# uzh-rpg/rpg_ramnet

Measured on AMD Instinct MI355X. Metric: depth samples/sec (346x260 cropped to 256x344, 5-bin grids, K=5 grids + 1 frame per sample; training step), higher is better.
Workload: dtype f32; 1 GPU; EventScape-shaped 346x260 -> 256x344 crop, 5 event bins, K=5, batch 8/GPU, seq-len 8, 1xMI355X-per-rank train, state=convgru, SI loss on [image,events4], Adam, backward-weights co-scheduled on a side stream, decoders on a second stream; global_batch=8, seq_len=8, parallelism=dp1

## Files before the change

rpg_ramnet_amd/csrc/conv_wgrad_wino24.hip:

```cpp
#include <stdlib.h>
#include "common.hpp"

namespace ramnet {

constexpr int G24_T = 8;

struct Wgrad24Params {
    const float *x, *g, *gm;
    float *dw, *dbias;
    int ldx, ldg, ldgm, Hp, Wp, H2, W2, Hc, Wc, Cin, Cout, tiles_x, tiles_y, ntiles, nbatch, ncob;
    size_t xbytes, gbytes, gmbytes;
};

template <bool GM, bool WCI>
__global__ void __launch_bounds__(512, 1) conv_wgrad_wino24_kernel(const Wgrad24Params p) {
    constexpr int G24_CI = WCI ? 64 : 32, G24_CO = WCI ? 32 : 64;
    constexpr int G24_V = 25 * G24_T * G24_CI, G24_Z = 25 * G24_T * G24_CO;
    extern __shared__ __attribute__((aligned(16))) float smem[];
    float *V = smem;
    float *Z = smem + 2 * G24_V;
    const int tid = threadIdx.x, lane = tid & 63;
    const int wave = __builtin_amdgcn_readfirstlane(tid >> 6);
    const int l31 = lane & 31, kk = lane >> 5;
    const int pg = wave >> 1, ch = wave & 1;
    const int p0 = pg == 0 ? 0 : 1 + 6 * pg;
    const int cls = blockIdx.z / p.ncob, cob = blockIdx.z % p.ncob;
    const int py = cls >> 1, px = cls & 1;
    const int c0 = blockIdx.y * G24_CI, n0 = cob * G24_CO;
    const bool vrole = WCI || wave < 4, zrole = !WCI || wave < 4;
    const int vt = (tid / G24_CI) & 7, vc = tid % G24_CI;
    const int zt = (tid / G24_CO) & 7, zc = tid % G24_CO;

    f32x16 acc[7];
#pragma unroll
    for (int i = 0; i < 7; ++i)
#pragma unroll
        for (int r = 0; r < 16; ++r) acc[i][r] = 0.f;

    float vraw[25], zraw[4];
    float bsum = 0.f;
    struct Walk { int tx, ty, b, T; };
    const int dT = G24_T * (int)gridDim.x;
    const int d_tx = dT % p.tiles_x, d_ty = (dT / p.tiles_x) % p.tiles_y, d_b = (dT / p.tiles_x) / p.tiles_y;
    auto walk_init = [&](Walk &w, int batch, int tile) {
        w.T = batch * G24_T + tile;
        int t = w.T;
        w.tx = t % p.tiles_x;
        t /= p.tiles_x;
        w.ty = t % p.tiles_y, w.b = t / p.tiles_y;
    };
    auto walk_step = [&](Walk &w, int adv) {
        w.T += adv * dT;
        w.tx += adv * d_tx;
        const int cx = w.tx >= p.tiles_x ? 1 : 0;
        w.tx -= cx * p.tiles_x;
        w.ty += adv * d_ty + cx;
        const int cy = w.ty >= p.tiles_y ? 1 : 0;
        w.ty -= cy * p.tiles_y;
        w.b += adv * d_b + cy;
    };
    Walk wv, wz;
    int lbv = 0, lbz = 0;
    const auto rx = wino_rsrc(p.x, (unsigned)min((size_t)p.xbytes, (size_t)WOOB));
    const auto rg = wino_rsrc(p.g, (unsigned)min((size_t)p.gbytes, (size_t)WOOB));
    const auto rgm = GM ? wino_rsrc(p.gm, (unsigned)min((size_t)p.gmbytes, (size_t)WOOB)) : rg;
    const bool vch_ok = c0 + vc < p.Cin, zch_ok = n0 + zc < p.Cout;
    const unsigned zch = (unsigned)(n0 + zc);
    const int rowB = p.Wp * p.ldx * 4, colB = p.ldx * 4;
    auto load_v = [&](int batch) {
        walk_step(wv, batch != lbv ? 1 : 0);
        lbv = batch;
        const unsigned base = (unsigned)(((wv.b * p.Hp + 2 * wv.ty + py) * p.Wp + 2 * wv.tx + px) * p.ldx + c0 + vc) * 4u;
        const unsigned lane_off = ((wv.T < p.ntiles) & vch_ok) ? base : WOOB;
#pragma unroll
        for (int r = 0; r < 5; ++r)
#pragma unroll
            for (int c = 0; c < 5; ++c)
                vraw[r * 5 + c] = __builtin_bit_cast(float, __builtin_amdgcn_raw_buffer_load_b32(rx, (int)(lane_off + (unsigned)(r * rowB)), c * colB, 0));
    };
    auto load_z = [&](int batch, bool count) {
        walk_step(wz, batch != lbz ? 1 : 0);
        lbz = batch;
        const bool tok = (wz.T < p.ntiles) & zch_ok;
#pragma unroll
        for (int a = 0; a < 2; ++a)
#pragma unroll
            for (int c = 0; c < 2; ++c) {
                const int oy = 2 * wz.ty + a, ox = 2 * wz.tx + c;
                const bool ok = tok & (oy < p.Hc) & (ox < p.Wc);
                const unsigned pix = (unsigned)((wz.b * p.H2 + 2 * oy + py) * p.W2 + 2 * ox + px);
                float v = __builtin_bit_cast(float, __builtin_amdgcn_raw_buffer_load_b32(rg, (int)(ok ? (pix * p.ldg + zch) * 4u : WOOB), 0, 0));
                if (GM) {
                    const float m = __builtin_bit_cast(float, __builtin_amdgcn_raw_buffer_load_b32(rgm, (int)(ok ? (pix * p.ldgm + zch) * 4u : WOOB), 0, 0));
                    v = m > 0.f ? v : 0.f;
                }
                zraw[a * 2 + c] = v;
                if (count) bsum += v;
            }
    };
    auto v_cols = [&]() {
#pragma unroll
        for (int c = 0; c < 5; ++c) {
            const float d0 = vraw[c], d1 = vraw[5 + c], d2 = vraw[10 + c], d3 = vraw[15 + c], d4 = vraw[20 + c];
            vraw[c] = 2.f * (d0 - d2) - d1 + d3;
            vraw[5 + c] = d3 - d2 - 2.f * d1;
            vraw[10 + c] = 2.f * d1 - 3.f * d2 + d3;
            vraw[15 + c] = d3 - d1;
            vraw[20 + c] = 2.f * (d1 - d3) - d2 + d4;
        }
    };
    auto v_row = [&](float *vbuf, int i) {
        const float d0 = vraw[i * 5], d1 = vraw[i * 5 + 1], d2 = vraw[i * 5 + 2], d3 = vraw[i * 5 + 3], d4 = vraw[i * 5 + 4];
        float *dst = vbuf + ((i * 5) * G24_T + vt) * G24_CI + vc;
        dst[0 * G24_T * G24_CI] = 2.f * (d0 - d2) - d1 + d3;
        dst[1 * G24_T * G24_CI] = d3 - d2 - 2.f * d1;
        dst[2 * G24_T * G24_CI] = 2.f * d1 - 3.f * d2 + d3;
        dst[3 * G24_T * G24_CI] = d3 - d1;
        dst[4 * G24_T * G24_CI] = 2.f * (d1 - d3) - d2 + d4;
    };
    auto z_row = [&](float *zbuf, int i) {
        float w0, w1;
        if (i == 0) w0 = zraw[0], w1 = zraw[1];
        if (i == 1) w0 = zraw[0] + zraw[2], w1 = zraw[1] + zraw[3];
        if (i == 2) w0 = zraw[0] - zraw[2], w1 = zraw[1] - zraw[3];
        if (i == 3) w0 = zraw[0] + 2.f * zraw[2], w1 = zraw[1] + 2.f * zraw[3];
        if (i == 4) w0 = zraw[2], w1 = zraw[3];
        float *dst = zbuf + ((i * 5) * G24_T + zt) * G24_CO + zc;
        dst[0 * G24_T * G24_CO] = w0;
        dst[1 * G24_T * G24_CO] = w0 + w1;
        dst[2 * G24_T * G24_CO] = w0 - w1;
        dst[3 * G24_T * G24_CO] = w0 + 2.f * w1;
        dst[4 * G24_T * G24_CO] = w1;
    };

    const int step = gridDim.x;
    int batch = blockIdx.x;
    if (batch < p.nbatch) {
        const int last = batch + ((p.nbatch - 1 - batch) / step) * step;
        walk_init(wv, batch, vt), walk_init(wz, batch, zt);
        lbv = lbz = batch;
        if (zrole) load_z(batch, true);
        if (vrole) load_v(batch);
        if (zrole) {
#pragma unroll
            for (int i = 0; i < 5; ++i) z_row(Z, i);
        }
        if (vrole) {
            v_cols();
#pragma unroll
            for (int i = 0; i < 5; ++i) v_row(V, i);
        }
        {
            const bool more = batch + step <= last;
            if (zrole) load_z(min(batch + step, last), more);
            if (vrole) load_v(min(batch + step, last));
        }
        __syncthreads();
        const int aoff = (kk * 4) * G24_CI + (WCI ? ch * 32 : 0) + l31, boff = (kk * 4) * G24_CO + (WCI ? 0 : ch * 32) + l31;
        int buf = 0;
        for (; batch <= last; batch += step, buf ^= 1) {
            const float *vb = V + buf * G24_V, *zb = Z + buf * G24_Z;
            float *vn = V + (buf ^ 1) * G24_V, *zn = Z + (buf ^ 1) * G24_Z;
            const int b2 = min(batch + 2 * step, last);
            const bool more2 = batch + 2 * step <= last;
#pragma unroll
            for (int q = 0; q < 7; ++q) {
                if (q < 6 || pg == 0) {
                    const int pos = p0 + q;
                    const float *ap = vb + pos * (G24_T * G24_CI) + aoff, *bp = zb + pos * (G24_T * G24_CO) + boff;
                    const float a0 = ap[0], a1 = ap[G24_CI], a2 = ap[2 * G24_CI], a3 = ap[3 * G24_CI];
                    const float b0 = bp[0], b1 = bp[G24_CO], b2v = bp[2 * G24_CO], b3 = bp[3 * G24_CO];
                    __builtin_amdgcn_sched_barrier(0);
                    acc[q] = __builtin_amdgcn_mfma_f32_32x32x2f32(a0, b0, acc[q], 0, 0, 0);
                    acc[q] = __builtin_amdgcn_mfma_f32_32x32x2f32(a1, b1, acc[q], 0, 0, 0);
                    __builtin_amdgcn_sched_barrier(0);
                    if (q == 0 && zrole) z_row(zn, 0), z_row(zn, 1), z_row(zn, 2);
                    if (q == 1 && zrole) z_row(zn, 3), z_row(zn, 4);
                    if (q == 2 && vrole) v_cols();
                    if (q == 3 && vrole) v_row(vn, 0), v_row(vn, 1), v_row(vn, 2);
                    if (q == 4 && vrole) v_row(vn, 3), v_row(vn, 4);
                    if (q == 4) {
                        if (zrole) load_z(b2, more2);
                        if (vrole) load_v(b2);
                    }
                    __builtin_amdgcn_sched_barrier(0);
                    acc[q] = __builtin_amdgcn_mfma_f32_32x32x2f32(a2, b2v, acc[q], 0, 0, 0);
                    acc[q] = __builtin_amdgcn_mfma_f32_32x32x2f32(a3, b3, acc[q], 0, 0, 0);
                    __builtin_amdgcn_sched_barrier(0);
                }
            }
            __syncthreads();
        }
    }

    const int n = n0 + (WCI ? 0 : ch * 32) + l31;
#pragma unroll
    for (int q = 0; q < 7; ++q) {
        if (q < 6 || pg == 0) {
#pragma unroll
            for (int r = 0; r < 16; ++r) {
                const int c = c0 + (WCI ? ch * 32 : 0) + (r & 3) + 8 * (r >> 2) + 4 * kk;
                if (c < p.Cin && n < p.Cout) atomicAdd(p.dw + (((size_t)cls * 25 + p0 + q) * p.Cin + c) * p.Cout + n, acc[q][r]);
            }
        }
    }
    if (p.dbias != nullptr && blockIdx.y == 0) {
        __syncthreads();
        float *red = smem;
        if (zrole) red[zt * G24_CO + zc] = bsum;
        __syncthreads();
        if (tid < G24_CO) {
            float t = 0.f;
            for (int g = 0; g < 8; ++g) t += red[g * G24_CO + tid];
            if (n0 + tid < p.Cout) atomicAdd(p.dbias + n0 + tid, t);
        }
    }
}

int launch_wgrad_wino24(const ramnet_wgrad_desc &d, hipStream_t st) {
    const bool wci = d.Cout % 64 != 0;
    const int G24_CI = wci ? 64 : 32, G24_CO = wci ? 32 : 64;
    RAMNET_CHECK_ARG(d.in_mode == RAMNET_IN_PLAIN && d.stride == 1 && d.C0 % G24_CI == 0 && d.Cout % 32 == 0);
    RAMNET_CHECK_ARG(d.Hin == d.Ho + 4 && d.Win == d.Wo + 4 && d.HoG == 2 * d.Ho && d.WoG == 2 * d.Wo && d.Ho >= 2 && d.Wo >= 2);
    Wgrad24Params q;
    q.x = d.x0, q.g = d.dout, q.gm = d.gmask, q.dw = d.dw, q.dbias = d.dbias;
    q.ldx = d.ld0, q.ldg = d.ldg, q.ldgm = d.ldgm, q.Hp = d.Hin, q.Wp = d.Win, q.H2 = d.HoG, q.W2 = d.WoG, q.Hc = d.Ho, q.Wc = d.Wo;
    q.Cin = d.C0, q.Cout = d.Cout;
    q.xbytes = (size_t)d.B * d.Hin * d.Win * d.ld0 * 4, q.gbytes = (size_t)d.B * d.HoG * d.WoG * d.ldg * 4;
    q.gmbytes = d.gmask ? (size_t)d.B * d.HoG * d.WoG * d.ldgm * 4 : 0;
    RAMNET_CHECK_ARG(2 * q.xbytes < WOOB && 2 * q.gbytes < WOOB && 2 * q.gmbytes < WOOB);
    q.tiles_x = cdiv(d.Wo, 2), q.tiles_y = cdiv(d.Ho, 2), q.ntiles = q.tiles_x * q.tiles_y * d.B, q.nbatch = cdiv(q.ntiles, G24_T);
    q.ncob = cdiv(d.Cout, G24_CO);
    const int gy = d.C0 / G24_CI, gz = q.ncob * 4;
    int splits = 256 / (gy * gz);
    if (splits > q.nbatch) splits = q.nbatch;
    if (splits < 1) splits = 1;
    const size_t lds = (size_t)2 * 25 * G24_T * (32 + 64) * sizeof(float);
    const dim3 grid(splits, gy, gz);
    auto go = [&](auto kern) -> int {
        RAMNET_FULL_LDS((kern));
        note_kernel("conv_wgrad_wino24_kernel<%d,%d>", d.gmask ? 1 : 0, (int)wci);
        hipLaunchKernelGGL(kern, grid, dim3(512), lds, st, q);
        return 0;
    };
    const int rc = wci ? (d.gmask ? go(conv_wgrad_wino24_kernel<true, true>) : go(conv_wgrad_wino24_kernel<false, true>))
                       : (d.gmask ? go(conv_wgrad_wino24_kernel<true, false>) : go(conv_wgrad_wino24_kernel<false, false>));
    if (rc) return rc;
    RAMNET_LAUNCH_CHECK();
    return 0;
}

}
```

Measured before the change: 247.5 samples/s.

## Software-pipeline LDS operand prefetch and spread transform stages across MFMA slots

Restructures the Winograd F(2,3) weight-gradient main loop so the LDS operands for the next group of MFMAs are fetched into registers ahead of time. The global-load and transform work (z/v loads, column/row transforms, mask application) is split into fine-grained slots interleaved between individual MFMAs instead of coarse chunks. The mid-loop barrier moves so the next buffer's reads overlap the current compute, and LDS base offsets are held as swapped opaque registers. It also adds compile-time ablation macros for profiling. The aim is to hide LDS and global latency behind MFMA issue, at the cost of more register pressure and scheduling complexity.

```diff
diff --git a/rpg_ramnet_amd/csrc/conv_wgrad_wino24.hip b/rpg_ramnet_amd/csrc/conv_wgrad_wino24.hip
--- a/rpg_ramnet_amd/csrc/conv_wgrad_wino24.hip
+++ b/rpg_ramnet_amd/csrc/conv_wgrad_wino24.hip
@@ -1,5 +1,21 @@
 #include <stdlib.h>
+#include <type_traits>
 #include "common.hpp"
+
+#ifndef RAMNET_ABL24
+#define RAMNET_ABL24 0
+#endif
+#define ABL24(bit) ((RAMNET_ABL24 & (bit)) != 0)
+#define RAMNET_OPQ(QQ) asm volatile("" : "+v"(QQ))
+#ifndef RAMNET_W24_AHEAD
+#define RAMNET_W24_AHEAD 1
+#endif
+#ifndef RAMNET_W24_ALT
+#define RAMNET_W24_ALT 1
+#endif
+#ifndef RAMNET_W24_SLOTS
+#define RAMNET_W24_SLOTS 1
+#endif
 
 namespace ramnet {
 
@@ -37,7 +53,7 @@
 #pragma unroll
         for (int r = 0; r < 16; ++r) acc[i][r] = 0.f;
 
-    float vraw[25], zraw[4];
+    float vraw[25], zraw[4], zmsk[4];
     float bsum = 0.f;
     struct Walk { int tx, ty, b, T; };
     const int dT = G24_T * (int)gridDim.x;
@@ -64,54 +80,56 @@
     const auto rx = wino_rsrc(p.x, (unsigned)min((size_t)p.xbytes, (size_t)WOOB));
     const auto rg = wino_rsrc(p.g, (unsigned)min((size_t)p.gbytes, (size_t)WOOB));
     const auto rgm = GM ? wino_rsrc(p.gm, (unsigned)min((size_t)p.gmbytes, (size_t)WOOB)) : rg;
-    const bool vch_ok = c0 + vc < p.Cin, zch_ok = n0 + zc < p.Cout;
+    const bool vch_ok = vrole & (c0 + vc < p.Cin), zch_ok = zrole & (n0 + zc < p.Cout);
     const unsigned zch = (unsigned)(n0 + zc);
     const int rowB = p.Wp * p.ldx * 4, colB = p.ldx * 4;
-    auto load_v = [&](int batch) {
+    unsigned vlo = WOOB;
+    bool ztok = false;
+    auto v_addr = [&](int batch) {
         walk_step(wv, batch != lbv ? 1 : 0);
         lbv = batch;
         const unsigned base = (unsigned)(((wv.b * p.Hp + 2 * wv.ty + py) * p.Wp + 2 * wv.tx + px) * p.ldx + c0 + vc) * 4u;
-        const unsigned lane_off = ((wv.T < p.ntiles) & vch_ok) ? base : WOOB;
-#pragma unroll
-        for (int r = 0; r < 5; ++r)
-#pragma unroll
-            for (int c = 0; c < 5; ++c)
-                vraw[r * 5 + c] = __builtin_bit_cast(float, __builtin_amdgcn_raw_buffer_load_b32(rx, (int)(lane_off + (unsigned)(r * rowB)), c * colB, 0));
-    };
-    auto load_z = [&](int batch, bool count) {
+        vlo = ((wv.T < p.ntiles) & vch_ok) ? base : WOOB;
+    };
+    auto v_load = [&](int k) {
+        const int r = k / 5, c = k % 5;
+        vraw[k] = __builtin_bit_cast(float, __builtin_amdgcn_raw_buffer_load_b32(rx, (int)(vlo + (unsigned)(r * rowB)), c * colB, 0));
+    };
+    auto z_addr = [&](int batch, bool count) {
         walk_step(wz, batch != lbz ? 1 : 0);
         lbz = batch;
-        const bool tok = (wz.T < p.ntiles) & zch_ok;
-#pragma unroll
-        for (int a = 0; a < 2; ++a)
-#pragma unroll
-            for (int c = 0; c < 2; ++c) {
-                const int oy = 2 * wz.ty + a, ox = 2 * wz.tx + c;
-                const bool ok = tok & (oy < p.Hc) & (ox < p.Wc);
-                const unsigned pix = (unsigned)((wz.b * p.H2 + 2 * oy + py) * p.W2 + 2 * ox + px);
-                float v = __builtin_bit_cast(float, __builtin_amdgcn_raw_buffer_load_b32(rg, (int)(ok ? (pix * p.ldg + zch) * 4u : WOOB), 0, 0));
-                if (GM) {
-                    const float m = __builtin_bit_cast(float, __builtin_amdgcn_raw_buffer_load_b32(rgm, (int)(ok ? (pix * p.ldgm + zch) * 4u : WOOB), 0, 0));
-                    v = m > 0.f ? v : 0.f;
-                }
-                zraw[a * 2 + c] = v;
-                if (count) bsum += v;
-            }
-    };
-    auto v_cols = [&]() {
-#pragma unroll
-        for (int c = 0; c < 5; ++c) {
-            const float d0 = vraw[c], d1 = vraw[5 + c], d2 = vraw[10 + c], d3 = vraw[15 + c], d4 = vraw[20 + c];
-            vraw[c] = 2.f * (d0 - d2) - d1 + d3;
-            vraw[5 + c] = d3 - d2 - 2.f * d1;
-            vraw[10 + c] = 2.f * d1 - 3.f * d2 + d3;
-            vraw[15 + c] = d3 - d1;
-            vraw[20 + c] = 2.f * (d1 - d3) - d2 + d4;
-        }
+        ztok = (wz.T < p.ntiles) & zch_ok & count;
+    };
+    auto z_load = [&](int a) {
+#pragma unroll
+        for (int c = 0; c < 2; ++c) {
+            const int oy = 2 * wz.ty + a, ox = 2 * wz.tx + c;
+            const bool ok = ztok & (oy < p.Hc) & (ox < p.Wc);
+            const unsigned pix = (unsigned)((wz.b * p.H2 + 2 * oy + py) * p.W2 + 2 * ox + px);
+            zraw[a * 2 + c] = __builtin_bit_cast(float, __builtin_amdgcn_raw_buffer_load_b32(rg, (int)(ok ? (pix * p.ldg + zch) * 4u : WOOB), 0, 0));
+            if (GM) zmsk[a * 2 + c] = __builtin_bit_cast(float, __builtin_amdgcn_raw_buffer_load_b32(rgm, (int)(ok ? (pix * p.ldgm + zch) * 4u : WOOB), 0, 0));
+        }
+    };
+    auto z_take = [&]() {
+#pragma unroll
+        for (int j = 0; j < 4; ++j) {
+            float v = zraw[j];
+            if (GM) v = zmsk[j] > 0.f ? v : 0.f;
+            zraw[j] = v;
+            bsum += v;
+        }
+    };
+    auto v_col = [&](int c) {
+        const float d0 = vraw[c], d1 = vraw[5 + c], d2 = vraw[10 + c], d3 = vraw[15 + c], d4 = vraw[20 + c];
+        vraw[c] = 2.f * (d0 - d2) - d1 + d3;
+        vraw[5 + c] = d3 - d2 - 2.f * d1;
+        vraw[10 + c] = 2.f * d1 - 3.f * d2 + d3;
+        vraw[15 + c] = d3 - d1;
+        vraw[20 + c] = 2.f * (d1 - d3) - d2 + d4;
     };
     auto v_row = [&](float *vbuf, int i) {
         const float d0 = vraw[i * 5], d1 = vraw[i * 5 + 1], d2 = vraw[i * 5 + 2], d3 = vraw[i * 5 + 3], d4 = vraw[i * 5 + 4];
-        float *dst = vbuf + ((i * 5) * G24_T + vt) * G24_CI + vc;
+        float *dst = vbuf + (i * 5) * G24_T * G24_CI;
         dst[0 * G24_T * G24_CI] = 2.f * (d0 - d2) - d1 + d3;
         dst[1 * G24_T * G24_CI] = d3 - d2 - 2.f * d1;
         dst[2 * G24_T * G24_CI] = 2.f * d1 - 3.f * d2 + d3;
@@ -125,7 +143,7 @@
         if (i == 2) w0 = zraw[0] - zraw[2], w1 = zraw[1] - zraw[3];
         if (i == 3) w0 = zraw[0] + 2.f * zraw[2], w1 = zraw[1] + 2.f * zraw[3];
         if (i == 4) w0 = zraw[2], w1 = zraw[3];
-        float *dst = zbuf + ((i * 5) * G24_T + zt) * G24_CO + zc;
+        float *dst = zbuf + (i * 5) * G24_T * G24_CO;
         dst[0 * G24_T * G24_CO] = w0;
         dst[1 * G24_T * G24_CO] = w0 + w1;
         dst[2 * G24_T * G24_CO] = w0 - w1;
@@ -133,70 +151,138 @@
         dst[4 * G24_T * G24_CO] = w1;
     };
 
+    const int vwo = vt * G24_CI + vc, zwo = zt * G24_CO + zc;
     const int step = gridDim.x;
     int batch = blockIdx.x;
     if (batch < p.nbatch) {
         const int last = batch + ((p.nbatch - 1 - batch) / step) * step;
         walk_init(wv, batch, vt), walk_init(wz, batch, zt);
         lbv = lbz = batch;
-        if (zrole) load_z(batch, true);
-        if (vrole) load_v(batch);
+        z_addr(batch, true), z_load(0), z_load(1);
+        v_addr(batch);
+#pragma unroll
+        for (int k = 0; k < 25; ++k) v_load(k);
+        z_take();
         if (zrole) {
 #pragma unroll
-            for (int i = 0; i < 5; ++i) z_row(Z, i);
+            for (int i = 0; i < 5; ++i) z_row(Z + zwo, i);
         }
         if (vrole) {
-            v_cols();
-#pragma unroll
-            for (int i = 0; i < 5; ++i) v_row(V, i);
+#pragma unroll
+            for (int c = 0; c < 5; ++c) v_col(c);
+#pragma unroll
+            for (int i = 0; i < 5; ++i) v_row(V + vwo, i);
         }
         {
             const bool more = batch + step <= last;
-            if (zrole) load_z(min(batch + step, last), more);
-            if (vrole) load_v(min(batch + step, last));
+            z_addr(min(batch + step, last), more), z_load(0), z_load(1);
+            v_addr(min(batch + step, last));
+#pragma unroll
+            for (int k = 0; k < 25; ++k) v_load(k);
         }
         __syncthreads();
-        const int aoff = (kk * 4) * G24_CI + (WCI ? ch * 32 : 0) + l31, boff = (kk * 4) * G24_CO + (WCI ? 0 : ch * 32) + l31;
-        int buf = 0;
-        for (; batch <= last; batch += step, buf ^= 1) {
-            const float *vb = V + buf * G24_V, *zb = Z + buf * G24_Z;
-            float *vn = V + (buf ^ 1) * G24_V, *zn = Z + (buf ^ 1) * G24_Z;
+        const int aoff = (p0 * G24_T + kk * 4) * G24_CI + (WCI ? ch * 32 : 0) + l31, boff = (p0 * G24_T + kk * 4) * G24_CO + (WCI ? 0 : ch * 32) + l31;
+        float oa[2][2][4], ob[2][2][4], oa6[4], ob6[4];
+        auto fetch = [&](const float *vs, const float *zs, int q0, int set, int r0, int r1) {
+#pragma unroll
+            for (int r = r0; r < r1; ++r) {
+                const int s = r >> 3, w = r & 7;
+                float &o = s == 2 ? (w < 4 ? oa6[w] : ob6[w - 4]) : (w < 4 ? oa[set][s][w] : ob[set][s][w - 4]);
+                if (ABL24(2)) RAMNET_OPQ(o);
+                else o = w < 4 ? vs[(q0 + s) * (G24_T * G24_CI) + w * G24_CI] : zs[(q0 + s) * (G24_T * G24_CO) + (w - 4) * G24_CO];
+            }
+        };
+        int vrc = aoff, vrn = G24_V + aoff, zrc = 2 * G24_V + boff, zrn = 2 * G24_V + G24_Z + boff;
+        int vwn = G24_V + vwo, vwc = vwo, zwn = 2 * G24_V + G24_Z + zwo, zwc = 2 * G24_V + zwo;
+        asm volatile("" : "+v"(vrc), "+v"(vrn), "+v"(zrc), "+v"(zrn), "+v"(vwn), "+v"(vwc), "+v"(zwn), "+v"(zwc));
+        if (ABL24(2)) {
+#pragma unroll
+            for (int i = 0; i < 16; ++i) (&oa[0][0][0])[i] = (&ob[0][0][0])[i] = oa6[i & 3] = ob6[i & 3] = 1.f;
+        }
+        if (RAMNET_W24_AHEAD) fetch(smem + vrc, smem + zrc, 0, 0, 0, 16);
+        do {
+            const float *va = smem + vrc, *za = smem + zrc;
+            const float *van = smem + vrn, *zan = smem + zrn;
+            float *vn = smem + vwn, *zn = smem + zwn;
             const int b2 = min(batch + 2 * step, last);
             const bool more2 = batch + 2 * step <= last;
-#pragma unroll
-            for (int q = 0; q < 7; ++q) {
-                if (q < 6 || pg == 0) {
-                    const int pos = p0 + q;
-                    const float *ap = vb + pos * (G24_T * G24_CI) + aoff, *bp = zb + pos * (G24_T * G24_CO) + boff;
-                    const float a0 = ap[0], a1 = ap[G24_CI], a2 = ap[2 * G24_CI], a3 = ap[3 * G24_CI];
-                    const float b0 = bp[0], b1 = bp[G24_CO], b2v = bp[2 * G24_CO], b3 = bp[3 * G24_CO];
+            auto stage = [&](int g) {
+                if (ABL24(1)) return;
+                if (RAMNET_W24_SLOTS) {
+                    if (g == 0) z_take();
+                    if (zrole && g < 5) z_row(zn, g);
+                    if (g == 5) z_addr(b2, more2), z_load(0);
+                    if (g == 6) z_load(1);
+                    if (vrole && g >= 5 && g < 10) v_col(g - 5);
+                    if (vrole && g >= 10 && g < 15) v_row(vn, g - 10);
+                    if (g == 10) v_addr(b2);
+#pragma unroll
+                    for (int k = 0; k < 25; ++k)
+                        if (g == 11 + k * 13 / 25) v_load(k);
+                } else {
+                    if (g == 1) z_take();
+                    if (zrole && g == 1) z_row(zn, 0), z_row(zn, 1), z_row(zn, 2);
+                    if (zrole && g == 3) z_row(zn, 3), z_row(zn, 4);
+                    if (vrole && g == 5) v_col(0), v_col(1), v_col(2), v_col(3), v_col(4);
+                    if (vrole && g == 9) v_row(vn, 0), v_row(vn, 1), v_row(vn, 2);
+                    if (vrole && g == 13) v_row(vn, 3), v_row(vn, 4);
+                    if (g == 17) {
+                        z_addr(b2, more2), z_load(0), z_load(1);
+                        v_addr(b2);
+#pragma unroll
+                        for (int k = 0; k < 25; ++k) v_load(k);
+                    }
+                }
+            };
+            auto group = [&](auto n_c, int q0, int set, int g0, const float *vsn, const float *zsn, int qn, bool third, int spread) {
+                constexpr int n = decltype(n_c)::value, M = 4 * n;
+                if (!RAMNET_W24_AHEAD) {
+                    fetch(va, za, q0, set, 0, 16);
+                    if (n == 3 && pg == 0) fetch(va, za, q0, set, 16, 24);
+                }
+#pragma unroll
+                for (int m = 0; m < M; ++m) {
+                    const int s = RAMNET_W24_ALT ? m % n : m / 4, k = RAMNET_W24_ALT ? m / n : m % 4;
+                    const bool skip = ABL24(16) && q0 + s >= 5;
                     __builtin_amdgcn_sched_barrier(0);
-                    acc[q] = __builtin_amdgcn_mfma_f32_32x32x2f32(a0, b0, acc[q], 0, 0, 0);
-                    acc[q] = __builtin_amdgcn_mfma_f32_32x32x2f32(a1, b1, acc[q], 0, 0, 0);
+                    if (s == 2) {
+                        if (pg == 0 && !skip) acc[q0 + 2] = __builtin_amdgcn_mfma_f32_32x32x2f32(oa6[k], ob6[k], acc[q0 + 2], 0, 0, 0);
+                    } else if (!skip) acc[q0 + s] = __builtin_amdgcn_mfma_f32_32x32x2f32(oa[set][s][k], ob[set][s][k], acc[q0 + s], 0, 0, 0);
                     __builtin_amdgcn_sched_barrier(0);
-                    if (q == 0 && zrole) z_row(zn, 0), z_row(zn, 1), z_row(zn, 2);
-                    if (q == 1 && zrole) z_row(zn, 3), z_row(zn, 4);
-                    if (q == 2 && vrole) v_cols();
-                    if (q == 3 && vrole) v_row(vn, 0), v_row(vn, 1), v_row(vn, 2);
-                    if (q == 4 && vrole) v_row(vn, 3), v_row(vn, 4);
-                    if (q == 4) {
-                        if (zrole) load_z(b2, more2);
-                        if (vrole) load_v(b2);
+                    if (RAMNET_W24_AHEAD) {
+                        if (m < spread) fetch(vsn, zsn, qn, set ^ 1, 16 * m / spread, 16 * (m + 1) / spread);
+                        if (third && pg == 0) fetch(vsn, zsn, qn, set ^ 1, 16 + m, 17 + m);
                     }
-                    __builtin_amdgcn_sched_barrier(0);
-                    acc[q] = __builtin_amdgcn_mfma_f32_32x32x2f32(a2, b2v, acc[q], 0, 0, 0);
-                    acc[q] = __builtin_amdgcn_mfma_f32_32x32x2f32(a3, b3, acc[q], 0, 0, 0);
-                    __builtin_amdgcn_sched_barrier(0);
+                    stage(g0 + m);
                 }
+            };
+            group(std::integral_constant<int, 2>{}, 0, 0, 0, va, za, 2, false, 8);
+            group(std::integral_constant<int, 2>{}, 2, 1, 8, va, za, 4, true, 8);
+            if (!ABL24(4)) __syncthreads();
+            group(std::integral_constant<int, 3>{}, 4, 0, 16, van, zan, 0, false, 8);
+            if (RAMNET_W24_AHEAD) {
+#pragma unroll
+                for (int i = 0; i < 8; ++i) (&oa[0][0][0])[i] = (&oa[1][0][0])[i], (&ob[0][0][0])[i] = (&ob[1][0][0])[i];
             }
-            __syncthreads();
-        }
+            int t;
+            t = vrc, vrc = vrn, vrn = t;
+            t = zrc, zrc = zrn, zrn = t;
+            t = vwc, vwc = vwn, vwn = t;
+            t = zwc, zwc = zwn, zwn = t;
+            batch += step;
+        } while (batch <= last);
     }
 
     const int n = n0 + (WCI ? 0 : ch * 32) + l31;
+    if (ABL24(8)) {
+        float t = 0.f;
+#pragma unroll
+        for (int q = 0; q < 7; ++q) t += acc[q][0] + acc[q][15];
+        if (t == 123.456f) p.dw[0] = t;
+    }
 #pragma unroll
     for (int q = 0; q < 7; ++q) {
-        if (q < 6 || pg == 0) {
+        if (!ABL24(8) && (q < 6 || pg == 0)) {
 #pragma unroll
             for (int r = 0; r < 16; ++r) {
                 const int c = c0 + (WCI ? ch * 32 : 0) + (r & 3) + 8 * (r >> 2) + 4 * kk;
@@ -240,6 +326,7 @@
     auto go = [&](auto kern) -> int {
         RAMNET_FULL_LDS((kern));
         note_kernel("conv_wgrad_wino24_kernel<%d,%d>", d.gmask ? 1 : 0, (int)wci);
+        if (ABL24(32)) return 0;
         hipLaunchKernelGGL(kern, grid, dim3(512), lds, st, q);
         return 0;
     };
```

After: 249.2 samples/s (median of 6 runs). No clear change (+0.7%).
